# AILab-UniFI/GNN-TableExtraction

Hardware: NVIDIA B200
Metric: page-graphs/sec (fwd+bwd train step) (higher is better)
Workload: dtype f32

## Files before the change

### gnn_tableextraction_b200/csrc/gte_spmm.cu

```cuda
#include "gte_common.cuh"
#include "gte_umma_ptx.cuh"

namespace gte {

template <int VEC>
struct Acc;
template <>
struct Acc<4> {
  float4 v;
  __device__ __forceinline__ void zero() { v = make_float4(0.f, 0.f, 0.f, 0.f); }
  __device__ __forceinline__ void fma(float w, const float4& x) {
    v.x = fmaf(w, x.x, v.x);
    v.y = fmaf(w, x.y, v.y);
    v.z = fmaf(w, x.z, v.z);
    v.w = fmaf(w, x.w, v.w);
  }
};
template <>
struct Acc<1> {
  float v;
  __device__ __forceinline__ void zero() { v = 0.f; }
  __device__ __forceinline__ void fma(float w, float x) { v = fmaf(w, x, v); }
};

// ... 367 lines not shown
    row[q] = (int64_t)cur.n0 + rl;
    if (cur.staged) {
      beg[q] = A.sptr[rl] - cur.e0;
      end[q] = A.sptr[rl + 1] - cur.e0;
    } else {
      beg[q] = __ldg(A.indptr + row[q]) - cur.e0;
      end[q] = __ldg(A.indptr + row[q] + 1) - cur.e0;
    }
  }
  float4 av[R][VV];
  float nrm[R];
#pragma unroll
  for (int q = 0; q < R; ++q) {
#pragma unroll
    for (int v = 0; v < VV; ++v) {
      av[q][v] = make_float4(0.f, 0.f, 0.f, 0.f);
      if (A.addend && on[v]) av[q][v] = __ldg(reinterpret_cast<const float4*>(A.addend + row[q] * A.ldadd + col[v]));
    }
    nrm[q] = 1.0f;
    if (A.mode == GTE_AGG_SUM_NORM) nrm[q] = cur.staged ? A.snrm[rl0 + q * NG] : __ldg(A.row_norm + row[q]);
  }
  float4 acc[R][VV];
#pragma unroll
  for (int q = 0; q < R; ++q)
#pragma unroll
    for (int v = 0; v < VV; ++v) acc[q][v] = make_float4(0.f, 0.f, 0.f, 0.f);
  if (cur.staged) {
    int32_t len = end[0] - beg[0];
    if (R == 2) len = max(len, end[R - 1] - beg[R - 1]);
    auto load_meta = [&](int32_t j, uint2 (&m)[R][U]) {
#pragma unroll
      for (int q = 0; q < R; ++q)
#pragma unroll
        for (int u = 0; u < U; ++u) {
          const int32_t e = beg[q] + j + u;
          m[q][u] = make_uint2(PK_OUTSIDE, 0u);
          if (e < end[q]) m[q][u] = MG ? __ldg(A.gpk + e) : A.spk[e];
        }
    };
    auto step = [&](const uint2 (&m)[R][U]) {
      float4 xv[R][U][VV];
#pragma unroll
      for (int q = 0; q < R; ++q)
#pragma unroll
        for (int u = 0; u < U; ++u) {
          const uint8_t* xr = A.xb + min(m[q][u].x, A.zrow) * ROW_BYTES;
#pragma unroll
          for (int v = 0; v < VV; ++v) xv[q][u][v] = *reinterpret_cast<const float4*>(xr + v * (G * 16));
        }
#pragma unroll
      for (int u = 0; u < U; ++u)
#pragma unroll
        for (int q = 0; q < R; ++q)
#pragma unroll
          for (int v = 0; v < VV; ++v) fma4(acc[q][v], __uint_as_float(m[q][u].y), xv[q][u][v]);
    };
    uint2 ma[R][U], mb[R][U];
    load_meta(0, ma);
    for (int32_t j = 0; j < len; j += 2 * U) {
      load_meta(j + U, mb);
      step(ma);
      if (j + U >= len) break;
      load_meta(j + 2 * U, ma);
      step(mb);
    }
  }
  if (A.slow) {
#pragma unroll 1
    for (int q = 0; q < R; ++q) {
      for (int32_t j = beg[q]; j < end[q]; ++j) {
        const int32_t c = __ldg(A.indices + cur.e0 + j);
        const int32_t sl = c - cur.n0;
        if (cur.staged && sl >= 0 && sl < cur.np) continue;
        float wt = A.w ? __ldg(A.w + (A.eid ? __ldg(A.eid + cur.e0 + j) : cur.e0 + j)) : 1.0f;
        if (A.pre_scale) wt *= __ldg(A.pre_scale + c);
#pragma unroll
        for (int v = 0; v < VV; ++v)
          if (on[v]) {
            const float4 xg = __ldg(reinterpret_cast<const float4*>(A.x + (int64_t)c * A.ldx + col[v]));
            if (q == 0) fma4(acc[0][v], wt, xg);
            else fma4(acc[R - 1][v], wt, xg);
          }
      }
    }
  }
#pragma unroll
  for (int q = 0; q < R; ++q) {
    const int32_t deg = end[q] - beg[q];
    const float d = (float)(deg > 1 ? deg : 1);
#pragma unroll
    for (int v = 0; v < VV; ++v) {
      if (!on[v]) continue;
      float4 r = acc[q][v];
      if (A.mode == GTE_AGG_MEAN) {
        r.x /= d; r.y /= d; r.z /= d; r.w /= d;
      } else if (A.mode == GTE_AGG_SUM_NORM) {
        r.x *= nrm[q]; r.y *= nrm[q]; r.z *= nrm[q]; r.w *= nrm[q];
      }
      if (A.addend) {
        r.x += av[q][v].x; r.y += av[q][v].y; r.z += av[q][v].z; r.w += av[q][v].w;
      }
      *reinterpret_cast<float4*>(A.y + row[q] * A.ldy + col[v]) = r;
    }
  }
}

template <int G, int V, int VV, bool MG>
__device__ __forceinline__ void pk_rows(const PkRowArgs& A) {
  constexpr int NG = PK_CONSUMERS / G;
  const int grp = threadIdx.x / G;
  for (int32_t rl0 = grp; rl0 < A.it.np; rl0 += 2 * NG) {
    if (rl0 + NG < A.it.np)
      pk_row_pass<G, V, VV, 2, MG>(A, rl0);
    else
      pk_row_pass<G, V, VV, 1, MG>(A, rl0);
  }
}

template <int G, int V, bool MG>
__global__ void __launch_bounds__(PK_THREADS, 1)
    k_spmm_paged_pk(const __grid_constant__ PkMaps maps, const int32_t* __restrict__ indptr,
                    const uint2* __restrict__ packed, const int32_t* __restrict__ page_flag,
                    const int32_t* __restrict__ indices, const int32_t* __restrict__ eid, const float* __restrict__ w,
                    const float* __restrict__ pre_scale, const float* __restrict__ row_norm, int mode,
                    const float* __restrict__ x, int64_t ldx, const float* __restrict__ addend, int64_t ldadd,
                    float* __restrict__ y, int64_t ldy, const int32_t* __restrict__ page_off, int32_t f, int32_t num_items,
                    int32_t nslices, int32_t items_per_cta, int32_t np_cap, int32_t ne_cap) {
  extern __shared__ __align__(128) uint8_t pk_smem[];
  constexpr int CS = G * V * 4;
  constexpr int ROW_BYTES = CS * 4;
  const PkStageLayout L = pk_layout(CS, np_cap, MG ? 0 : ne_cap);
  const uint32_t stage_bytes = L.stage_bytes();
  const uint32_t smem0 = (uint32_t)__cvta_generic_to_shared(pk_smem);
  const uint32_t bars = smem0 + 2 * stage_bytes;
  const uint32_t off_pk = L.x_bytes, off_ptr = off_pk + L.pk_bytes, off_nrm = off_ptr + L.ptr_bytes,
                 off_info = off_nrm + L.nrm_bytes;
  const int tid = threadIdx.x;

  const int item_beg = blockIdx.x * items_per_cta;
  const int item_end = min(num_items, item_beg + items_per_cta);
  if (item_beg >= item_end) return;
  if (tid == 0) {
    mbar_init(bars, 2);
    mbar_init(bars + 8, 2);
    mbar_init(bars + 16, PK_CONSUMERS / 32);
    mbar_init(bars + 24, PK_CONSUMERS / 32);
    fence_barrier_init();
    tma_prefetch_desc(&maps.big);
    tma_prefetch_desc(&maps.small);
  }
  for (int i = tid; i < 2 * (ROW_BYTES / 4); i += PK_THREADS) {
    const int st = i / (ROW_BYTES / 4), c = i % (ROW_BYTES / 4);
    reinterpret_cast<float*>(pk_smem + (size_t)st * stage_bytes + L.x_bytes - ROW_BYTES)[c] = 0.f;
  }
  __syncthreads();

  if (tid >= PK_CONSUMERS) {
    const int pl = tid - PK_CONSUMERS;
    auto load_item = [&](int item) {
      PkItem it = {0, 0, 0, 0, 0, 0, 0, 0};
      if (item < item_end) {
        const int page = item / nslices;
        it.c0 = (item - page * nslices) * CS;
        it.n0 = __ldg(page_off + page);
        it.np = __ldg(page_off + page + 1) - it.n0;
        it.e0 = __ldg(indptr + it.n0);
        it.ne = __ldg(indptr + it.n0 + it.np) - it.e0;
        it.flag = __ldg(page_flag + page);
        it.staged = (it.np <= np_cap && (MG || it.ne <= ne_cap)) ? 1 : 0;
      }
      return it;
    };
    PkItem it = load_item(item_beg);
    for (int item = item_beg, s = 0, k = 0; item < item_end; ++item, s ^= 1, ++k) {
      const PkItem nxt = load_item(item + 1);
      if (k >= 2) mbar_wait_backoff(bars + 16 + s * 8, (uint32_t)((k >> 1) - 1) & 1u);
      uint8_t* sbase = pk_smem + (size_t)s * stage_bytes;
      const uint32_t sx = smem0 + s * stage_bytes;
      const uint32_t bar = bars + s * 8;
      if (pl == 0) {
        *reinterpret_cast<PkItem*>(sbase + off_info) = it;
        if (it.staged) {
          const int nbig = it.np / PK_BOX_BIG;
          const int nsmall = (it.np - nbig * PK_BOX_BIG + PK_BOX_SMALL - 1) / PK_BOX_SMALL;
          const int e_lo = it.e0 & ~1;
          const uint32_t pk_copy = (!MG && it.ne > 0) ? (uint32_t)((it.e0 + it.ne - e_lo + 1) & ~1) * 8u : 0u;
          mbar_expect_tx(bar, (uint32_t)(nbig * PK_BOX_BIG + nsmall * PK_BOX_SMALL) * ROW_BYTES + pk_copy);
          for (int b = 0; b < nbig; ++b)
            tma_load_2d(sx + b * PK_BOX_BIG * ROW_BYTES, &maps.big, bar, it.c0, it.n0 + b * PK_BOX_BIG);
          for (int b = 0; b < nsmall; ++b)
            tma_load_2d(sx + (nbig * PK_BOX_BIG + b * PK_BOX_SMALL) * ROW_BYTES, &maps.small, bar, it.c0,
                        it.n0 + nbig * PK_BOX_BIG + b * PK_BOX_SMALL);
          if (pk_copy) bulk_load_1d(sx + off_pk, packed + e_lo, pk_copy, bar);
        } else {
          mbar_arrive(bar);
        }
      }
      if (it.staged) {
        int32_t* sptr = reinterpret_cast<int32_t*>(sbase + off_ptr);
        float* snrm = reinterpret_cast<float*>(sbase + off_nrm);
        const int32_t* ip = indptr + it.n0;
        for (int i = pl; i <= it.np; i += 32) sptr[i] = __ldg(ip + i);
        if (mode == GTE_AGG_SUM_NORM) {
          const float* nr = row_norm + it.n0;
          for (int i = pl; i < it.np; i += 32) snrm[i] = __ldg(nr + i);
        }
      }
      if (addend) {
        for (int i = pl; i < it.np * 2; i += 32) {
          const int col = it.c0 + (i & 1) * 32;
          if (col < f) asm volatile("prefetch.global.L2 [%0];" ::"l"(addend + (int64_t)(it.n0 + (i >> 1)) * ldadd + col));
        }
      }
      __syncwarp();
      if (pl == 0) mbar_arrive(bar);
      it = nxt;
    }
  } else {
    const int lane = tid % G;
    PkRowArgs A;
    A.zrow = L.x_bytes / ROW_BYTES - 1;
    A.indptr = indptr; A.indices = indices; A.eid = eid; A.w = w; A.pre_scale = pre_scale; A.row_norm = row_norm;
    A.mode = mode; A.x = x; A.ldx = ldx; A.addend = addend; A.ldadd = ldadd; A.y = y; A.ldy = ldy; A.f = f;
    for (int item = item_beg, s = 0, k = 0; item < item_end; ++item, s ^= 1, ++k) {
      mbar_wait(bars + s * 8, (uint32_t)(k >> 1) & 1u);
      const uint8_t* sbase = pk_smem + (size_t)s * stage_bytes;
      A.it = *reinterpret_cast<const PkItem*>(sbase + off_info);
      A.xb = sbase + lane * 16;
      A.spk = reinterpret_cast<const uint2*>(sbase + off_pk) + (A.it.e0 & 1);
      A.gpk = packed + A.it.e0;
      A.sptr = reinterpret_cast<const int32_t*>(sbase + off_ptr);
      A.snrm = reinterpret_cast<const float*>(sbase + off_nrm);
      A.slow = !A.it.staged || A.it.flag != 0;
      if (V == 2 && A.it.c0 + G * 4 >= f)
        pk_rows<G, V, 1, MG>(A);
      else
        pk_rows<G, V, V, MG>(A);
      __syncwarp();
      if ((tid & 31) == 0) mbar_arrive(bars + 16 + s * 8);
    }
  }
}

static size_t pk_smem_bytes(int cs, int32_t np_cap, int32_t ne_cap) {
  return 2 * (size_t)pk_layout(cs, np_cap, ne_cap).stage_bytes() + 32;
}

constexpr size_t PK_SMEM_MAX = 227 * 1024;

static void pk_pick(int32_t f, int32_t np_cap, int32_t ne_cap, int* G, int* V, int* MG) {
  const int fv = (f + 3) / 4;
  *G = 0;
  *V = 0;
  *MG = 0;
  struct Cand { int cs, mg; };
  const Cand wide[] = {{64, 0}, {32, 0}, {64, 1}, {32, 1}, {16, 0}, {16, 1}};
  const Cand mid[] = {{32, 0}, {32, 1}, {16, 0}, {16, 1}};
  const Cand narrow[] = {{16, 0}, {16, 1}};
  const Cand* c = fv > 8 ? wide : (fv > 4 ? mid : narrow);
  const int nc = fv > 8 ? 6 : (fv > 4 ? 4 : 2);
  for (int i = 0; i < nc; ++i) {
    if (pk_smem_bytes(c[i].cs, np_cap, c[i].mg ? 0 : ne_cap) <= PK_SMEM_MAX) {
      *G = c[i].cs == 16 ? 4 : 8;
      *V = c[i].cs == 64 ? 2 : 1;
      *MG = c[i].mg;
      return;
    }
  }
}

template <int G, int V, bool MG>
static int launch_spmm_paged_pk(const int32_t* indptr, const uint2* packed, const int32_t* page_flag,
                                const int32_t* indices, const int32_t* eid, const float* w, const float* pre_scale,
                                const float* row_norm, int mode, const float* x, int64_t ldx, const float* addend,
                                int64_t ldadd, float* y, int64_t ldy, const int32_t* page_off, int32_t num_pages,
                                int32_t np_cap, int32_t ne_cap, int32_t n_rows, int32_t f, cudaStream_t st) {
  constexpr int CS = G * V * 4;
  const size_t smem = pk_smem_bytes(CS, np_cap, MG ? 0 : ne_cap);
  if (int rc = ensure_dynamic_smem(reinterpret_cast<const void*>(&k_spmm_paged_pk<G, V, MG>), smem, "k_spmm_paged_pk")) return rc;
  int occ = 1;
  GTE_CHECK_CUDA(cudaOccupancyMaxActiveBlocksPerMultiprocessor(&occ, k_spmm_paged_pk<G, V, MG>, PK_THREADS, smem),
                 "k_spmm_paged_pk(occupancy)");
  if (occ < 1) occ = 1;
  PkMaps maps;
  {
    int rc = make_tmap_2d(&maps.big, x, n_rows, f, ldx, CS, PK_BOX_BIG, CU_TENSOR_MAP_SWIZZLE_NONE);
    if (rc) return rc;
    rc = make_tmap_2d(&maps.small, x, n_rows, f, ldx, CS, PK_BOX_SMALL, CU_TENSOR_MAP_SWIZZLE_NONE);
    if (rc) return rc;
  }
  const int nslices = (int)ceil_div64((f + 3) / 4, G * V);
  const int64_t items = (int64_t)num_pages * nslices;
  GTE_CHECK_ARG(items < (int64_t)1 << 31, "gte_spmm_paged_packed: too many (page, slice) items");
  int grid = (int)(items < (int64_t)sm_count() * occ ? items : (int64_t)sm_count() * occ);
  const int per = (int)ceil_div64(items, grid);
  grid = (int)ceil_div64(items, per);
  k_spmm_paged_pk<G, V, MG><<<grid, PK_THREADS, smem, st>>>(maps, indptr, packed, page_flag, indices, eid, w, pre_scale, row_norm,
                                                       mode, x, ldx, addend, ldadd, y, ldy, page_off, f, (int32_t)items,
                                                       nslices, per, np_cap, ne_cap);
  GTE_CHECK_LAUNCH("k_spmm_paged_pk");
  return GTE_OK;
}

}

using namespace gte;

extern "C" int gte_spmm(const int32_t* indptr, const int32_t* indices, const float* w, const float* pre_scale,
                        const float* row_norm, int mode, const float* x, int64_t ldx, const float* addend,
                        int64_t ldadd, float* y, int64_t ldy, int32_t n_rows, int32_t f, gte_stream_t stream) {
  GTE_CHECK_ARG(n_rows >= 0 && f >= 0, "gte_spmm: negative size");
  GTE_CHECK_ARG(mode == GTE_AGG_SUM || mode == GTE_AGG_SUM_NORM || mode == GTE_AGG_MEAN, "gte_spmm: bad mode %d", mode);
  if (n_rows == 0 || f == 0) return GTE_OK;
  GTE_CHECK_ARG(indptr && indices && x && y, "gte_spmm: null argument");
  GTE_CHECK_ARG(mode != GTE_AGG_SUM_NORM || row_norm, "gte_spmm: SUM_NORM needs row_norm");
  GTE_CHECK_ARG(ldx >= f && ldy >= f && (!addend || ldadd >= f), "gte_spmm: leading dimension < f");
  GTE_CHECK_ARG(x != y, "gte_spmm: x and y must not alias");
  cudaStream_t st = as_stream(stream);
  const bool vec = aligned16(x) && aligned16(y) && (ldx % 4 == 0) && (ldy % 4 == 0) &&
                   (!addend || (aligned16(addend) && ldadd % 4 == 0));
#define GTE_SPMM_GO(VEC, G, C) \
  return launch_spmm<VEC, G, C>(indptr, indices, w, pre_scale, row_norm, mode, x, ldx, addend, ldadd, y, ldy, n_rows, f, st)
  if (vec) {
    const int nv = (f + 3) / 4;
    if (nv <= 4) GTE_SPMM_GO(4, 4, 1);
    if (nv <= 8) GTE_SPMM_GO(4, 8, 1);
    if (nv <= 16) GTE_SPMM_GO(4, 16, 1);
    if (nv <= 32) GTE_SPMM_GO(4, 32, 1);
    if (nv <= 64) GTE_SPMM_GO(4, 32, 2);
    if (nv <= 96) GTE_SPMM_GO(4, 32, 3);
    GTE_SPMM_GO(4, 32, 4);
  } else {
    if (f <= 4) GTE_SPMM_GO(1, 4, 1);
    if (f <= 8) GTE_SPMM_GO(1, 8, 1);
    if (f <= 16) GTE_SPMM_GO(1, 16, 1);
    if (f <= 32) GTE_SPMM_GO(1, 32, 1);
    if (f <= 64) GTE_SPMM_GO(1, 32, 2);
    GTE_SPMM_GO(1, 32, 4);
  }
#undef GTE_SPMM_GO
}

extern "C" int gte_spmm_paged(const int32_t* indptr, const int32_t* indices, const float* w, const float* pre_scale,
                              const float* row_norm, int mode, const float* x, int64_t ldx, const float* addend,
                              int64_t ldadd, float* y, int64_t ldy, const int32_t* page_off, int32_t num_pages,
                              int32_t max_page_nodes, int32_t max_page_edges, int32_t n_rows, int32_t f,
                              gte_stream_t stream) {
  GTE_CHECK_ARG(n_rows >= 0 && f >= 0 && num_pages >= 0 && max_page_nodes >= 0 && max_page_edges >= 0,
                "gte_spmm_paged: negative size");
  GTE_CHECK_ARG(mode == GTE_AGG_SUM || mode == GTE_AGG_SUM_NORM || mode == GTE_AGG_MEAN, "gte_spmm_paged: bad mode %d", mode);
  if (n_rows == 0 || f == 0 || num_pages == 0) return GTE_OK;
  GTE_CHECK_ARG(indptr && indices && x && y && page_off, "gte_spmm_paged: null argument");
  GTE_CHECK_ARG(mode != GTE_AGG_SUM_NORM || row_norm, "gte_spmm_paged: SUM_NORM needs row_norm");
  GTE_CHECK_ARG(ldx >= f && ldy >= f && (!addend || ldadd >= f), "gte_spmm_paged: leading dimension < f");
  GTE_CHECK_ARG(x != y, "gte_spmm_paged: x and y must not alias");
  const bool vec = aligned16(x) && aligned16(y) && (ldx % 4 == 0) && (ldy % 4 == 0) &&
                   (!addend || (aligned16(addend) && ldadd % 4 == 0));
  const size_t budget = 110 * 1024;
  int G = 0;
  const int fv = (f + 3) / 4;
  for (int g : {32, 16, 8}) {
    if (paged_smem_bytes(g, max_page_nodes, max_page_edges) <= budget) {
      G = g;
      break;
    }
  }
  while (G > 8 && G / 2 >= fv) G /= 2;
  if (!vec || G == 0)
    return gte_spmm(indptr, indices, w, pre_scale, row_norm, mode, x, ldx, addend, ldadd, y, ldy, n_rows, f, stream);
  cudaStream_t st = as_stream(stream);
#define GTE_PAGED_GO(GG)                                                                                               \
  return launch_spmm_paged<GG>(indptr, indices, w, pre_scale, row_norm, mode, x, ldx, addend, ldadd, y, ldy, page_off, \
                               num_pages, max_page_nodes, max_page_edges, f, st)
  if (G == 32) GTE_PAGED_GO(32);
  if (G == 16) GTE_PAGED_GO(16);
  GTE_PAGED_GO(8);
#undef GTE_PAGED_GO
}

extern "C" int gte_paged_pack_edges(const int32_t* indptr, const int32_t* indices, const int32_t* eid, const float* w,
                                    const float* pre_scale, const int32_t* page_off, int32_t num_pages,
                                    uint64_t* packed, int32_t* page_flag, gte_stream_t stream) {
  GTE_CHECK_ARG(num_pages >= 0, "gte_paged_pack_edges: negative size");
  if (num_pages == 0) return GTE_OK;
  GTE_CHECK_ARG(indptr && indices && page_off && packed && page_flag, "gte_paged_pack_edges: null argument");
  GTE_CHECK_ARG((reinterpret_cast<uintptr_t>(packed) & 7u) == 0, "gte_paged_pack_edges: packed must be 8-byte aligned");
  k_paged_pack_edges<<<num_pages, 256, 0, as_stream(stream)>>>(indptr, indices, eid, w, pre_scale, page_off,
                                                              reinterpret_cast<uint2*>(packed), page_flag);
  GTE_CHECK_LAUNCH("k_paged_pack_edges");
  return GTE_OK;
}

extern "C" size_t gte_spmm_paged_packed_smem_bytes(int32_t max_page_nodes, int32_t max_page_edges, int32_t f) {
  if (max_page_nodes < 0 || max_page_edges < 0 || f <= 0) return 0;
  int G, V, MG;
  pk_pick(f, max_page_nodes, max_page_edges, &G, &V, &MG);
  return G ? pk_smem_bytes(G * V * 4, max_page_nodes, MG ? 0 : max_page_edges) : 0;
}

extern "C" int gte_spmm_paged_packed(const int32_t* indptr, const uint64_t* packed, const int32_t* page_flag,
                                     const int32_t* indices, const int32_t* eid, const float* w, const float* pre_scale,
                                     const float* row_norm, int mode, const float* x, int64_t ldx, const float* addend,
                                     int64_t ldadd, float* y, int64_t ldy, const int32_t* page_off, int32_t num_pages,
                                     int32_t max_page_nodes, int32_t max_page_edges, int32_t n_rows, int32_t f,
                                     gte_stream_t stream) {
  GTE_CHECK_ARG(n_rows >= 0 && f >= 0 && num_pages >= 0 && max_page_nodes >= 0 && max_page_edges >= 0,
                "gte_spmm_paged_packed: negative size");
  GTE_CHECK_ARG(mode == GTE_AGG_SUM || mode == GTE_AGG_SUM_NORM || mode == GTE_AGG_MEAN, "gte_spmm_paged_packed: bad mode %d",
                mode);
  if (n_rows == 0 || f == 0 || num_pages == 0) return GTE_OK;
  GTE_CHECK_ARG(indptr && packed && page_flag && indices && x && y && page_off, "gte_spmm_paged_packed: null argument");
  GTE_CHECK_ARG(mode != GTE_AGG_SUM_NORM || row_norm, "gte_spmm_paged_packed: SUM_NORM needs row_norm");
  GTE_CHECK_ARG(ldx >= f && ldy >= f && (!addend || ldadd >= f), "gte_spmm_paged_packed: leading dimension < f");
  GTE_CHECK_ARG(x != y, "gte_spmm_paged_packed: x and y must not alias");
  const bool vec = aligned16(x) && aligned16(y) && (ldx % 4 == 0) && (ldy % 4 == 0) &&
                   (!addend || (aligned16(addend) && ldadd % 4 == 0));
  int G, V, MG;
  pk_pick(f, max_page_nodes, max_page_edges, &G, &V, &MG);
  if (!vec || G == 0)
    return fail(GTE_ERR_UNSUPPORTED,
                "gte_spmm_paged_packed: operands not 16-byte aligned or pages too large to stage (query "
                "gte_spmm_paged_packed_smem_bytes first); use gte_spmm_paged");
  cudaStream_t st = as_stream(stream);
  const uint2* pk = reinterpret_cast<const uint2*>(packed);
#define GTE_PK_GO(GG, VV, MM)                                                                                              \
  return launch_spmm_paged_pk<GG, VV, MM>(indptr, pk, page_flag, indices, eid, w, pre_scale, row_norm, mode, x, ldx,     \
                                          addend, ldadd, y, ldy, page_off, num_pages, max_page_nodes, max_page_edges,    \
                                          n_rows, f, st)
  if (G == 8 && V == 2 && !MG) GTE_PK_GO(8, 2, false);
  if (G == 8 && V == 2) GTE_PK_GO(8, 2, true);
  if (G == 8 && !MG) GTE_PK_GO(8, 1, false);
  if (G == 8) GTE_PK_GO(8, 1, true);
  if (!MG) GTE_PK_GO(4, 1, false);
  GTE_PK_GO(4, 1, true);
#undef GTE_PK_GO
}
```

### gnn_tableextraction_b200/csrc/gte_umma2.cu

```cuda
#include "gte_umma_args.cuh"

#include <cuda.h>

namespace gte {

#ifdef GTE_EXPERIMENTS
__device__ long long g_umma2_dbg[148 * 16 * 8];
__device__ long long g_umma2_acc[148 * 16];
#define U2_T0() const long long t0__ = clock64()
#define U2_ACC(var) var += clock64() - t0__
#define U2_PUT(slot, v) do { if (blockIdx.x < 148) g_umma2_acc[blockIdx.x * 16 + (slot)] = (v); } while (0)
#else
#define U2_T0()
#define U2_ACC(var)
#define U2_PUT(slot, v)
#endif

constexpr int U2_THREADS = 448;
constexpr int U2_EPI_WARP0 = 4;
constexpr int U2_EPI_WARPS = 8;
constexpr int U2_SPLIT_WARPS = 4;
constexpr int U2_PREFETCH = 8;
constexpr int U2_EPI_BUF = 4096;
constexpr int U2_MAX_STAGES = 6;
constexpr size_t U2_SMEM_MAX = 227 * 1024;

struct U2Layout {
  uint32_t bh_bytes, stage_bytes, epi_off, par_off, stat_off, bar_off, tmem_off, total;
};
__host__ __device__ inline U2Layout u2_layout(int BN, int stages, int epi_bufs) {
  U2Layout L;
  L.bh_bytes = (uint32_t)(BN / 2) * 128u;
  L.stage_bytes = 2u * UM_A_BYTES + 2u * L.bh_bytes;
  L.epi_off = (uint32_t)stages * L.stage_bytes;
  L.par_off = L.epi_off + U2_EPI_WARPS * U2_EPI_BUF * (uint32_t)epi_bufs;
  L.stat_off = L.par_off + 3u * UM_MAX_BN * 4u;
  L.bar_off = L.stat_off + 2u * 2u * 128u * 8u;
  L.tmem_off = L.bar_off + (3u * U2_MAX_STAGES + 4u) * 8u;
  L.total = L.tmem_off + 16u;
  return L;
}

template <bool SPLIT>
__global__ void __cluster_dims__(2, 1, 1) __launch_bounds__(U2_THREADS, 1)
    k_umma_gemm_pair(const __grid_constant__ UmmaArgs P) {
  extern __shared__ __align__(1024) uint8_t smem_raw[];
  uint8_t* base = smem_raw + ((1024u - (smem_u32(smem_raw) & 1023u)) & 1023u);
  const U2Layout L = u2_layout(P.BN, P.stages, P.epi_bufs);
  const int S = P.stages;
  uint8_t* const tiles = base;
  auto sA_hi_p = [&](int s) { return tiles + s * L.stage_bytes; };
  auto sA_lo_p = [&](int s) { return tiles + s * L.stage_bytes + UM_A_BYTES; };
  auto sB_hi_p = [&](int s) { return tiles + s * L.stage_bytes + 2 * UM_A_BYTES; };
  auto sB_lo_p = [&](int s) { return tiles + s * L.stage_bytes + 2 * UM_A_BYTES + L.bh_bytes; };
  uint8_t* const s_stage = base + L.epi_off;
  float* const s_bias = reinterpret_cast<float*>(base + L.par_off);
  float* const s_gamma = s_bias + UM_MAX_BN;
  float* const s_beta = s_gamma + UM_MAX_BN;
  float2* const s_stat = reinterpret_cast<float2*>(base + L.stat_off);
  uint64_t* const bars = reinterpret_cast<uint64_t*>(base + L.bar_off);
  uint64_t* const bar_full = bars;
  uint64_t* const bar_ready = bars + U2_MAX_STAGES;
  uint64_t* const bar_empty = bars + 2 * U2_MAX_STAGES;
  uint64_t* const bar_tfull = bars + 3 * U2_MAX_STAGES;
  uint64_t* const bar_tempty = bar_tfull + 2;
  uint32_t* const s_tmem = reinterpret_cast<uint32_t*>(base + L.tmem_off);

  const uint32_t rank = cluster_ctarank();
  const int warp = threadIdx.x >> 5;
  const int lane = threadIdx.x & 31;
  const int m_tiles = (P.M + UM_BM - 1) / UM_BM;
  const int m_pairs = (m_tiles + 1) / 2;
  const int total = m_pairs * P.ngroups;
  const int cluster_id = blockIdx.x >> 1, nclusters = gridDim.x >> 1;
  const int kb_total = P.kblocks[0] + (P.nseg > 1 ? P.kblocks[1] : 0);
#ifdef GTE_EXPERIMENTS
  auto stamp = [&](int t, int slot) {
    if (P.dbg && blockIdx.x < 148) {
      const int i = (t - cluster_id) / nclusters;
      if (i < 16) g_umma2_dbg[(blockIdx.x * 16 + i) * 8 + slot] = clock64();
    }
  };
#else
  auto stamp = [](int, int) {};
#endif

  for (int i = threadIdx.x; i < UM_MAX_BN; i += U2_THREADS) {
    s_bias[i] = (P.bias && i < P.bias_n) ? P.bias[i] : 0.f;
    s_gamma[i] = (P.gamma && i < P.N) ? P.gamma[i] : 1.f;
    s_beta[i] = (P.beta && i < P.N) ? P.beta[i] : 0.f;
  }
  if (warp == 0 && lane == 0) {
    for (int s = 0; s < S; ++s) {
      mbar_init(smem_u32(&bar_full[s]), 1);
      mbar_init(smem_u32(&bar_ready[s]), 2 * U2_SPLIT_WARPS);
      mbar_init(smem_u32(&bar_empty[s]), 1);
    }
    for (int a = 0; a < 2; ++a) {
      mbar_init(smem_u32(&bar_tfull[a]), 1);
      mbar_init(smem_u32(&bar_tempty[a]), SPLIT ? 2 * U2_EPI_WARPS : U2_EPI_WARPS);
    }
    fence_barrier_init();
    for (int s = 0; s < P.nseg; ++s) tma_prefetch_desc(&P.tmA[s]);
    for (int gq = 0; gq < P.ngroups; ++gq)
      for (int s = 0; s < P.nseg; ++s) {
        tma_prefetch_desc(&P.tmBhi[gq][s]);
        tma_prefetch_desc(&P.tmBlo[gq][s]);
      }
  }
  if (warp == 1) tmem_alloc_pair(smem_u32(s_tmem), 512);
  tc_fence_before();
  __syncthreads();
  cluster_sync_all();
  tc_fence_after();
  const uint32_t tmem_base = *s_tmem;

  if (warp == 0) {
    if (lane == 0) {
      int stage = 0;
      uint32_t phase = 0;
      const int b_row0 = (int)rank * (P.BN >> 1);
      int pf_t = cluster_id, pf_seg = 0, pf_kb = 0;
      auto pf_step = [&]() {
        if (pf_t >= total) return;
        tma_prefetch_2d(&P.tmA[pf_seg], pf_kb * UM_BK, (2 * (pf_t / P.ngroups) + (int)rank) * UM_BM);
        if (++pf_kb >= P.kblocks[pf_seg]) {
          pf_kb = 0;
          if (++pf_seg >= P.nseg) {
            pf_seg = 0;
            pf_t += nclusters;
          }
        }
      };
#ifdef GTE_EXPERIMENTS
      if (P.dbg & 32) pf_t = total;
#endif
      for (int i = 0; i < U2_PREFETCH; ++i) pf_step();
      long long w_pe = 0, n_kb = 0;
      const long long t_begin = clock64();
      (void)w_pe; (void)n_kb; (void)t_begin;
      for (int t = cluster_id; t < total; t += nclusters) {
        const int mt = 2 * (t / P.ngroups) + (int)rank, grp = t % P.ngroups;
        stamp(t, 7);
        for (int seg = 0; seg < P.nseg; ++seg) {
          for (int kb = 0; kb < P.kblocks[seg]; ++kb) {
            pf_step();
            ++n_kb;
            {
              U2_T0();
              mbar_wait_cluster_backoff(smem_u32(&bar_empty[stage]), phase ^ 1);
              U2_ACC(w_pe);
            }
            const uint32_t fb = smem_u32(&bar_full[stage]);
            mbar_expect_tx(fb, (uint32_t)UM_A_BYTES + 2u * L.bh_bytes);
            tma_load_2d(smem_u32(sA_hi_p(stage)), &P.tmA[seg], fb, kb * UM_BK, mt * UM_BM);
            tma_load_2d(smem_u32(sB_hi_p(stage)), &P.tmBhi[grp][seg], fb, kb * UM_BK, b_row0);
            tma_load_2d(smem_u32(sB_lo_p(stage)), &P.tmBlo[grp][seg], fb, kb * UM_BK, b_row0);
            if (++stage == S) { stage = 0; phase ^= 1; }
          }
        }
      }
      U2_PUT(0, clock64() - t_begin);
      U2_PUT(1, w_pe);
      U2_PUT(9, n_kb);
    }
  } else if (warp == 1) {
    if (rank == 0 && lane == 0) {
      const uint32_t idesc = (1u << 4) | (2u << 7) | (2u << 10) | ((uint32_t)(P.BN >> 3) << 17) | ((uint32_t)(256 >> 4) << 24);
      int stage = 0;
      uint32_t phase = 0;
      int acc = 0;
      uint32_t acc_phase = 0;
      constexpr int nacc = SPLIT ? 1 : 2;
      long long w_mt = 0, w_mr = 0;
      const long long t_begin = clock64();
      (void)w_mt; (void)w_mr; (void)t_begin;
      for (int t = cluster_id; t < total; t += nclusters) {
        stamp(t, 4);
        {
          U2_T0();
          mbar_wait_cluster(smem_u32(&bar_tempty[acc]), acc_phase ^ 1);
          U2_ACC(w_mt);
        }
        tc_fence_after();
        stamp(t, 5);
        const uint32_t d_tmem = tmem_base + (uint32_t)(acc * UM_ACC_STRIDE);
        const uint32_t d_cross = SPLIT ? tmem_base + UM_ACC_STRIDE : d_tmem;
        for (int kb = 0; kb < kb_total; ++kb) {
          {
            U2_T0();
            mbar_wait_cluster(smem_u32(&bar_ready[stage]), phase);
            U2_ACC(w_mr);
          }
          tc_fence_after();
          const uint64_t dah = make_desc_k_sw128(smem_u32(sA_hi_p(stage)));
          const uint64_t dal = make_desc_k_sw128(smem_u32(sA_lo_p(stage)));
          const uint64_t dbh = make_desc_k_sw128(smem_u32(sB_hi_p(stage)));
          const uint64_t dbl = make_desc_k_sw128(smem_u32(sB_lo_p(stage)));
#pragma unroll
          for (int k = 0; k < UM_BK / 8; ++k) {
            const uint64_t adv = (uint64_t)((k * 8 * 4) >> 4);
            umma_tf32_pair(d_cross, dal + adv, dbh + adv, idesc, (kb | k) != 0 ? 1u : 0u);
            umma_tf32_pair(d_cross, dah + adv, dbl + adv, idesc, 1u);
            umma_tf32_pair(d_tmem, dah + adv, dbh + adv, idesc, (SPLIT && (kb | k) == 0) ? 0u : 1u);
          }
          umma_commit_pair(smem_u32(&bar_empty[stage]));
          if (++stage == S) { stage = 0; phase ^= 1; }
        }
        stamp(t, 6);
        umma_commit_pair(smem_u32(&bar_tfull[acc]));
        if (++acc == nacc) { acc = 0; acc_phase ^= 1; }
      }
      U2_PUT(4, w_mt);
      U2_PUT(5, w_mr);
      U2_PUT(6, clock64() - t_begin);
    }
  } else if (warp < U2_EPI_WARP0 || warp >= U2_EPI_WARP0 + U2_EPI_WARPS) {
    const int t = ((warp < U2_EPI_WARP0) ? warp - 2 : warp - (U2_EPI_WARP0 + U2_EPI_WARPS) + 2) * 32 + lane;
    const uint32_t ready_leader = mapa_shared(smem_u32(&bar_ready[0]), 0);
    int stage = 0;
    uint32_t phase = 0;
    long long w_sf = 0, w_sw = 0;
    (void)w_sf; (void)w_sw;
    for (int tile = cluster_id; tile < total; tile += nclusters) {
      for (int kb = 0; kb < kb_total; ++kb) {
        {
          U2_T0();
          mbar_wait_backoff(smem_u32(&bar_full[stage]), phase);
          U2_ACC(w_sf);
        }
        U2_T0();
        const float4* hi = reinterpret_cast<const float4*>(sA_hi_p(stage));
        float4* lo = reinterpret_cast<float4*>(sA_lo_p(stage));
#pragma unroll
        for (int i = 0; i < UM_A_BYTES / 16 / (U2_SPLIT_WARPS * 32); ++i) {
          const int idx = t + U2_SPLIT_WARPS * 32 * i;
          const float4 v = hi[idx];
          float4 l;
          l.x = tf32_rna(v.x - tf32_hi(v.x)); l.y = tf32_rna(v.y - tf32_hi(v.y));
          l.z = tf32_rna(v.z - tf32_hi(v.z)); l.w = tf32_rna(v.w - tf32_hi(v.w));
          lo[idx] = l;
        }
        fence_proxy_async();
        __syncwarp();
        if (lane == 0) mbar_arrive_cluster(ready_leader + (uint32_t)stage * 8u);
        U2_ACC(w_sw);
        if (++stage == S) { stage = 0; phase ^= 1; }
      }
    }
    if (t == 0) {
      U2_PUT(2, w_sf);
      U2_PUT(3, w_sw);
    }
  } else {
    const int ew = warp - U2_EPI_WARP0;
    const int q = warp & 3;
    const int half = ew >> 2;
    uint8_t* const stb = s_stage + ew * U2_EPI_BUF * P.epi_bufs;
    const int nbuf = P.epi_bufs;
    const uint32_t tempty_leader = mapa_shared(smem_u32(&bar_tempty[0]), 0);
    int store_seq = 0;
    int acc = 0;
    uint32_t acc_phase = 0;
    int par = 0;
    constexpr int nacc = SPLIT ? 1 : 2;
    const int nchunks = (P.N + 31) / 32;
    const int c_split = SPLIT ? (nchunks + 1) / 2 : nchunks;
    const int c_beg = (SPLIT && half) ? c_split : 0, c_end = (SPLIT && half) ? nchunks : c_split;
    const int cols_a = min(P.N, c_split * 32);
    const float n_a = (float)cols_a, n_b = (float)(P.N - cols_a), n_all = (float)P.N;
    const float my_n = (SPLIT && half) ? n_b : n_a;
    long long w_et = 0, w_ew = 0;
    (void)w_et; (void)w_ew;
    int it = 0;
    for (int t = cluster_id; t < total; t += nclusters, ++it) {
      const int mt = 2 * (t / P.ngroups) + (int)rank, grp = t % P.ngroups;
      if constexpr (!SPLIT) {
        if ((it & 1) != half) continue;
        acc = half;
        acc_phase = (uint32_t)(it >> 1) & 1u;
      }
      if (ew == 0 && lane == 0) stamp(t, 0);
      {
        U2_T0();
        mbar_wait_cluster_backoff(smem_u32(&bar_tfull[acc]), acc_phase);
        U2_ACC(w_et);
      }
      U2_T0();
      tc_fence_after();
      if (ew == 0 && lane == 0) stamp(t, 1);
      const uint32_t t_base = tmem_base + ((uint32_t)(q * 32) << 16) + (uint32_t)(acc * UM_ACC_STRIDE);
      const int64_t row0 = (int64_t)mt * UM_BM + q * 32;
      const bool rows_live = row0 < (int64_t)P.M;
      const bool store_z = P.out[grp] != nullptr && rows_live;
      const bool store_y = P.y != nullptr && rows_live;
      float x[32];
      const int rows_valid = rows_live ? (int)min((int64_t)32, (int64_t)P.M - row0) : 0;
      auto put_chunk = [&](const CUtensorMap* map, float* dst, int64_t ld, int c) {
#ifdef GTE_EXPERIMENTS
        if (P.dbg & 2) return;
#endif
        if (P.tma_store == 2)
          epi_store_chunk_lsu(stb, x, dst + row0 * ld + c * 32, ld, rows_valid, P.N - c * 32);
        else
          epi_store_chunk_tma(stb, nbuf, store_seq, x, map, c * 32, (int32_t)row0);
      };
#define load_chunk(c) epi_load_chunk<SPLIT>(t_base + (c) * 32, s_bias + (c) * 32, x)
      if (P.fuse_ln) {
        float shift = 0.f, s1 = 0.f, s2 = 0.f;
        for (int c = c_beg; c < c_end; ++c) {
          load_chunk(c);
          const int nv = min(32, P.N - c * 32);
          if (c == c_beg) {
            float s0 = 0.f;
#pragma unroll
            for (int j = 0; j < 32; ++j) s0 += (j < nv) ? x[j] : 0.f;
            shift = s0 / (float)nv;
          }
#ifdef GTE_EXPERIMENTS
          if (P.dbg & 8) { s1 += x[0]; s2 += x[1]; } else
#endif
          if (nv == 32) {
#pragma unroll
            for (int j = 0; j < 32; ++j) {
              const float d = x[j] - shift;
              s1 += d;
              s2 = fmaf(d, d, s2);
            }
          } else {
#pragma unroll
            for (int j = 0; j < 32; ++j) {
              const float d = (j < nv) ? x[j] - shift : 0.f;
              s1 += d;
              s2 = fmaf(d, d, s2);
            }
          }
          if (store_z) put_chunk(&P.tmOut[grp], P.out[grp], P.ldo[grp], c);
        }
        float mh = 0.f, m2h = 0.f;
        if (my_n > 0.f) {
          mh = shift + s1 / my_n;
          m2h = fmaxf(s2 - s1 * s1 / my_n, 0.f);
        }
        float mean = mh, m2 = m2h;
        if constexpr (SPLIT) {
          float2* const st = s_stat + (par * 2) * 128 + q * 32 + lane;
          st[half * 128] = make_float2(mh, m2h);
          asm volatile("bar.sync %0, 64;" ::"r"(1 + q) : "memory");
          const float2 pa = st[0], pb = st[128];
          par ^= 1;
          mean = pa.x;
          m2 = pa.y;
          if (n_b > 0.f) {
            const float delta = pb.x - pa.x;
            mean = pa.x + delta * (n_b / n_all);
            m2 = pa.y + pb.y + delta * delta * (n_a * n_b / n_all);
          }
        }
        const float rstd = 1.0f / sqrtf(m2 / n_all + P.eps);
        if (!SPLIT || half == 0) {
          const int64_t grow = row0 + lane;
          if (grow < P.M) {
            P.mean[grow] = mean;
            P.rstd[grow] = rstd;
          }
        }
        if (ew == 0 && lane == 0) stamp(t, 2);
        for (int c = c_beg; c < c_end; ++c) {
          load_chunk(c);
#ifdef GTE_EXPERIMENTS
          if (!(P.dbg & 4))
#endif
          epi_norm_act(x, s_gamma + c * 32, s_beta + c * 32, true, P.relu != 0, mean, rstd);
          if (store_y) put_chunk(&P.tmY, P.y, P.ldy, c);
        }
      } else {
        if (ew == 0 && lane == 0) stamp(t, 2);
        for (int c = c_beg; c < c_end; ++c) {
          load_chunk(c);
          if (store_z) put_chunk(&P.tmOut[grp], P.out[grp], P.ldo[grp], c);
          if (P.y != nullptr) {
            epi_norm_act(x, s_gamma + c * 32, s_beta + c * 32, false, P.relu != 0, 0.f, 1.f);
            if (store_y) put_chunk(&P.tmY, P.y, P.ldy, c);
          }
        }
      }
#undef load_chunk
      if (ew == 0 && lane == 0) stamp(t, 3);
      tc_fence_before();
      __syncwarp();
      if (lane == 0) mbar_arrive_cluster(tempty_leader + (uint32_t)acc * 8u);
      if constexpr (SPLIT) {
        if (++acc == nacc) { acc = 0; acc_phase ^= 1; }
      }
      U2_ACC(w_ew);
    }
    if (ew == 0 && lane == 0) {
      U2_PUT(7, w_et);
      U2_PUT(8, w_ew);
    }
    if (lane == 0) tma_store_wait_all();
  }
  tc_fence_before();
  __syncwarp();
  __syncthreads();
  cluster_sync_all();
  if (warp == 1) {
    tc_fence_after();
    tmem_dealloc_pair(tmem_base, 512);
  }
}

static void u2_pick(int BN, int kb_total, int* stages, int* epi_bufs) {
  *stages = 0;
  *epi_bufs = 1;
  if (kb_total <= 2) {
    for (int b = 4; b >= 1; --b)
      if (1024 + (size_t)u2_layout(BN, 2, b).total <= U2_SMEM_MAX) {
        *stages = 2;
        *epi_bufs = b;
        return;
      }
    return;
  }
  for (int s = U2_MAX_STAGES; s >= 2; --s)
    if (1024 + (size_t)u2_layout(BN, s, 1).total <= U2_SMEM_MAX) {
      *stages = s;
      if (1024 + (size_t)u2_layout(BN, s, 2).total <= U2_SMEM_MAX) *epi_bufs = 2;
      return;
    }
}

bool umma_pair_supported(const UmmaArgs& a) {
  const int m_tiles = (a.M + UM_BM - 1) / UM_BM;
  int st = 0, eb = 0;
  u2_pick(a.BN, 3, &st, &eb);
  return a.tma_store != 0 && m_tiles >= 2 && a.BN % 16 == 0 && a.BN >= 16 && a.BN <= UM_MAX_BN && sm_count() >= 2 && st >= 2;
}

int launch_umma_pair(UmmaArgs& a, cudaStream_t st) {
  if (int rc = setup_weight_maps(a, a.BN / 2)) return rc;
  const int kb_total = a.kblocks[0] + (a.nseg > 1 ? a.kblocks[1] : 0);
  int stages = 0, epi_bufs = 1;
  u2_pick(a.BN, kb_total, &stages, &epi_bufs);
  if (stages < 2) return fail(GTE_ERR_UNSUPPORTED, "k_umma_gemm_pair: BN=%d does not fit shared memory", a.BN);
  a.stages = stages;
  a.epi_bufs = epi_bufs;
  if (tuning(GTE_TUNE_EPI_STORE) == 1) a.tma_store = 2;
  const size_t smem = 1024 + (size_t)u2_layout(a.BN, a.stages, a.epi_bufs).total;
  if (int rc = ensure_dynamic_smem(reinterpret_cast<const void*>(&k_umma_gemm_pair<true>), smem, "k_umma_gemm_pair")) return rc;
  if (int rc = ensure_dynamic_smem(reinterpret_cast<const void*>(&k_umma_gemm_pair<false>), smem, "k_umma_gemm_pair")) return rc;
  const int m_tiles = (a.M + UM_BM - 1) / UM_BM;
  const int total = ((m_tiles + 1) / 2) * a.ngroups;
  int clusters = sm_count() / 2;
  if (clusters > total) clusters = total;
  if (clusters < 1) return GTE_OK;
  if (kb_total > 2 && tuning(GTE_TUNE_UMMA_SPLIT) != 0)
    k_umma_gemm_pair<true><<<2 * clusters, U2_THREADS, smem, st>>>(a);
  else
    k_umma_gemm_pair<false><<<2 * clusters, U2_THREADS, smem, st>>>(a);
  GTE_CHECK_LAUNCH("k_umma_gemm_pair");
  return GTE_OK;
}

int umma_pair_debug_times(int64_t* out_host, int32_t count) {
#ifdef GTE_EXPERIMENTS
  if (count == 148 * 16) {
    GTE_CHECK_CUDA(cudaMemcpyFromSymbol(out_host, g_umma2_acc, (size_t)count * 8), "gte_umma_debug_times");
    return GTE_OK;
  }
  GTE_CHECK_CUDA(cudaMemcpyFromSymbol(out_host, g_umma2_dbg, (size_t)count * 8), "gte_umma_debug_times");
  return GTE_OK;
#else
  (void)out_host;
  (void)count;
  return fail(GTE_ERR_UNSUPPORTED, "built without -DGTE_EXPERIMENTS");
#endif
}

}
```

Before: 390,900.

## Add narrow-feature paged SpMM kernel and grouped 128-row TMA epilogue stores

Adds a dedicated SpMM kernel for feature widths up to 16 that stages a whole page's node features, packed edges and row pointers into shared memory with cp.async. Each node row is then handled by four threads using float4 lanes, which avoids the wider slice-based packed kernel that wastes lanes on narrow features. Separately, the paired UMMA GEMM epilogue gains a grouped TMA store mode: the four epilogue warps write a swizzled 128x32 tile and one thread issues the store after a named barrier. This replaces per-warp 32-row stores and rebuilds the output tensor maps with a 128-row box. The costs are an extra barrier in the epilogue and a different shared-buffer indexing scheme.

```diff
diff --git a/gnn_tableextraction_b200/csrc/gte_spmm.cu b/gnn_tableextraction_b200/csrc/gte_spmm.cu
--- a/gnn_tableextraction_b200/csrc/gte_spmm.cu
+++ b/gnn_tableextraction_b200/csrc/gte_spmm.cu
@@ -693,6 +693,155 @@
   return GTE_OK;
 }
 
+constexpr int NW_THREADS = 256;
+constexpr int NW_ROWS = NW_THREADS / 4;
+
+struct NwLayout {
+  uint32_t x_bytes, pk_bytes, ptr_bytes;
+  __host__ __device__ uint32_t total() const { return x_bytes + pk_bytes + ptr_bytes; }
+};
+__host__ __device__ inline NwLayout nw_layout(int32_t np_cap, int32_t ne_cap) {
+  NwLayout l;
+  l.x_bytes = ((uint32_t)np_cap + 1) * 64;
+  l.pk_bytes = (uint32_t)ne_cap * 8;
+  l.ptr_bytes = (((uint32_t)np_cap + 1) * 4 + 15u) & ~15u;
+  return l;
+}
+
+__device__ __forceinline__ void cp_async_16_zfill(void* dst, const void* src, uint32_t src_bytes) {
+  asm volatile("cp.async.cg.shared.global [%0], [%1], 16, %2;" ::"r"((uint32_t)__cvta_generic_to_shared(dst)), "l"(src),
+               "r"(src_bytes)
+               : "memory");
+}
+__device__ __forceinline__ void cp_async_8(void* dst, const void* src) {
+  asm volatile("cp.async.ca.shared.global [%0], [%1], 8;" ::"r"((uint32_t)__cvta_generic_to_shared(dst)), "l"(src) : "memory");
+}
+__device__ __forceinline__ void cp_async_4(void* dst, const void* src) {
+  asm volatile("cp.async.ca.shared.global [%0], [%1], 4;" ::"r"((uint32_t)__cvta_generic_to_shared(dst)), "l"(src) : "memory");
+}
+
+__global__ void __launch_bounds__(NW_THREADS)
+    k_spmm_narrow(const int32_t* __restrict__ indptr, const uint2* __restrict__ packed, const int32_t* __restrict__ page_flag,
+                  const int32_t* __restrict__ indices, const int32_t* __restrict__ eid, const float* __restrict__ w,
+                  const float* __restrict__ pre_scale, const float* __restrict__ row_norm, int mode,
+                  const float* __restrict__ x, int64_t ldx, const float* __restrict__ addend, int64_t ldadd,
+                  float* __restrict__ y, int64_t ldy, const int32_t* __restrict__ page_off, int32_t f, int32_t np_cap,
+                  int32_t ne_cap) {
+  extern __shared__ __align__(16) uint8_t nw_smem[];
+  const NwLayout L = nw_layout(np_cap, ne_cap);
+  float4* sx = reinterpret_cast<float4*>(nw_smem);
+  uint2* spk = reinterpret_cast<uint2*>(nw_smem + L.x_bytes);
+  int32_t* sptr = reinterpret_cast<int32_t*>(nw_smem + L.x_bytes + L.pk_bytes);
+  const int tid = threadIdx.x;
+  const int page = blockIdx.x;
+  const int32_t n0 = __ldg(page_off + page), np = __ldg(page_off + page + 1) - n0;
+  const int32_t e0 = __ldg(indptr + n0), ne = __ldg(indptr + n0 + np) - e0;
+  const bool staged = np <= np_cap && ne <= ne_cap;
+  const bool slow = !staged || __ldg(page_flag + page) != 0;
+  if (staged) {
+    for (int i = tid; i < np * 4; i += NW_THREADS) {
+      const int r = i >> 2, c = (i & 3) * 4;
+      const int valid = min(max(f - c, 0), 4);
+      cp_async_16_zfill(sx + i, x + (int64_t)(n0 + r) * ldx + (valid ? c : 0), (uint32_t)valid * 4u);
+    }
+    for (int i = tid; i < ne; i += NW_THREADS) cp_async_8(spk + i, packed + e0 + i);
+    for (int i = tid; i <= np; i += NW_THREADS) cp_async_4(sptr + i, indptr + n0 + i);
+    asm volatile("cp.async.commit_group;" ::: "memory");
+    if (tid < 4) sx[np_cap * 4 + tid] = make_float4(0.f, 0.f, 0.f, 0.f);
+  }
+  const int lane = tid & 3;
+  const int col = lane * 4;
+  const bool on = col < f;
+  const uint32_t zrow = (uint32_t)np_cap;
+  auto row_ops = [&](int32_t rl, float4& a, float& nr) {
+    a = make_float4(0.f, 0.f, 0.f, 0.f);
+    nr = 1.0f;
+    if (rl >= np) return;
+    const int64_t row = (int64_t)n0 + rl;
+    if (addend && on) a = __ldg(reinterpret_cast<const float4*>(addend + row * ldadd + col));
+    if (mode == GTE_AGG_SUM_NORM) nr = __ldg(row_norm + row);
+  };
+  float4 av_next;
+  float nrm_next;
+  row_ops(tid >> 2, av_next, nrm_next);
+  if (staged) asm volatile("cp.async.wait_group 0;" ::: "memory");
+  __syncthreads();
+
+  for (int32_t rl = tid >> 2; rl < np; rl += NW_ROWS) {
+    const int64_t row = (int64_t)n0 + rl;
+    const float4 av = av_next;
+    const float nrm = nrm_next;
+    row_ops(rl + NW_ROWS, av_next, nrm_next);
+    int32_t beg, end;
+    if (staged) {
+      beg = sptr[rl] - e0;
+      end = sptr[rl + 1] - e0;
+    } else {
+      beg = __ldg(indptr + row) - e0;
+      end = __ldg(indptr + row + 1) - e0;
+    }
+    float4 acc = make_float4(0.f, 0.f, 0.f, 0.f);
+    if (staged) {
+      int32_t j = beg;
+      for (; j + 4 <= end; j += 4) {
+        const uint2 m0 = spk[j], m1 = spk[j + 1], m2 = spk[j + 2], m3 = spk[j + 3];
+        const float4 x0 = sx[min(m0.x, zrow) * 4 + lane];
+        const float4 x1 = sx[min(m1.x, zrow) * 4 + lane];
+        const float4 x2 = sx[min(m2.x, zrow) * 4 + lane];
+        const float4 x3 = sx[min(m3.x, zrow) * 4 + lane];
+        fma4(acc, __uint_as_float(m0.y), x0);
+        fma4(acc, __uint_as_float(m1.y), x1);
+        fma4(acc, __uint_as_float(m2.y), x2);
+        fma4(acc, __uint_as_float(m3.y), x3);
+      }
+      for (; j < end; ++j) {
+        const uint2 m = spk[j];
+        fma4(acc, __uint_as_float(m.y), sx[min(m.x, zrow) * 4 + lane]);
+      }
+    }
+    if (slow && on) {
+      for (int32_t j = beg; j < end; ++j) {
+        const int32_t c = __ldg(indices + e0 + j);
+        const int32_t sl = c - n0;
+        if (staged && sl >= 0 && sl < np) continue;
+        float wt = w ? __ldg(w + (eid ? __ldg(eid + e0 + j) : e0 + j)) : 1.0f;
+        if (pre_scale) wt *= __ldg(pre_scale + c);
+        fma4(acc, wt, __ldg(reinterpret_cast<const float4*>(x + (int64_t)c * ldx + col)));
+      }
+    }
+    if (!on) continue;
+    if (mode == GTE_AGG_MEAN) {
+      const int32_t deg = end - beg;
+      const float d = (float)(deg > 1 ? deg : 1);
+      acc.x /= d; acc.y /= d; acc.z /= d; acc.w /= d;
+    } else if (mode == GTE_AGG_SUM_NORM) {
+      acc.x *= nrm; acc.y *= nrm; acc.z *= nrm; acc.w *= nrm;
+    }
+    if (addend) {
+      acc.x += av.x; acc.y += av.y; acc.z += av.z; acc.w += av.w;
+    }
+    *reinterpret_cast<float4*>(y + row * ldy + col) = acc;
+  }
+}
+
+static size_t nw_smem_bytes(int32_t np_cap, int32_t ne_cap) {
+  if ((int64_t)np_cap * 64 + (int64_t)ne_cap * 8 > (int64_t)PK_SMEM_MAX) return 0;
+  const size_t b = nw_layout(np_cap, ne_cap).total();
+  return b <= PK_SMEM_MAX ? b : 0;
+}
+
+static int launch_spmm_narrow(const int32_t* indptr, const uint2* packed, const int32_t* page_flag, const int32_t* indices,
+                              const int32_t* eid, const float* w, const float* pre_scale, const float* row_norm, int mode,
+                              const float* x, int64_t ldx, const float* addend, int64_t ldadd, float* y, int64_t ldy,
+                              const int32_t* page_off, int32_t num_pages, int32_t np_cap, int32_t ne_cap, int32_t f,
+                              size_t smem, cudaStream_t st) {
+  if (int rc = ensure_dynamic_smem(reinterpret_cast<const void*>(&k_spmm_narrow), smem, "k_spmm_narrow")) return rc;
+  k_spmm_narrow<<<num_pages, NW_THREADS, smem, st>>>(indptr, packed, page_flag, indices, eid, w, pre_scale, row_norm, mode,
+                                                     x, ldx, addend, ldadd, y, ldy, page_off, f, np_cap, ne_cap);
+  GTE_CHECK_LAUNCH("k_spmm_narrow");
+  return GTE_OK;
+}
+
 }
 
 using namespace gte;
@@ -784,6 +933,9 @@
 
 extern "C" size_t gte_spmm_paged_packed_smem_bytes(int32_t max_page_nodes, int32_t max_page_edges, int32_t f) {
   if (max_page_nodes < 0 || max_page_edges < 0 || f <= 0) return 0;
+  if (f <= 16) {
+    if (const size_t b = nw_smem_bytes(max_page_nodes, max_page_edges)) return b;
+  }
   int G, V, MG;
   pk_pick(f, max_page_nodes, max_page_edges, &G, &V, &MG);
   return G ? pk_smem_bytes(G * V * 4, max_page_nodes, MG ? 0 : max_page_edges) : 0;
@@ -806,14 +958,19 @@
   GTE_CHECK_ARG(x != y, "gte_spmm_paged_packed: x and y must not alias");
   const bool vec = aligned16(x) && aligned16(y) && (ldx % 4 == 0) && (ldy % 4 == 0) &&
                    (!addend || (aligned16(addend) && ldadd % 4 == 0));
+  cudaStream_t st = as_stream(stream);
+  const uint2* pk = reinterpret_cast<const uint2*>(packed);
+  if (f <= 16 && vec) {
+    if (const size_t smem = nw_smem_bytes(max_page_nodes, max_page_edges))
+      return launch_spmm_narrow(indptr, pk, page_flag, indices, eid, w, pre_scale, row_norm, mode, x, ldx, addend, ldadd,
+                                y, ldy, page_off, num_pages, max_page_nodes, max_page_edges, f, smem, st);
+  }
   int G, V, MG;
   pk_pick(f, max_page_nodes, max_page_edges, &G, &V, &MG);
   if (!vec || G == 0)
     return fail(GTE_ERR_UNSUPPORTED,
                 "gte_spmm_paged_packed: operands not 16-byte aligned or pages too large to stage (query "
                 "gte_spmm_paged_packed_smem_bytes first); use gte_spmm_paged");
-  cudaStream_t st = as_stream(stream);
-  const uint2* pk = reinterpret_cast<const uint2*>(packed);
 #define GTE_PK_GO(GG, VV, MM)                                                                                              \
   return launch_spmm_paged_pk<GG, VV, MM>(indptr, pk, page_flag, indices, eid, w, pre_scale, row_norm, mode, x, ldx,     \
                                           addend, ldadd, y, ldy, page_off, num_pages, max_page_nodes, max_page_edges,    \
diff --git a/gnn_tableextraction_b200/csrc/gte_umma2.cu b/gnn_tableextraction_b200/csrc/gte_umma2.cu
--- a/gnn_tableextraction_b200/csrc/gte_umma2.cu
+++ b/gnn_tableextraction_b200/csrc/gte_umma2.cu
@@ -39,6 +39,29 @@
   L.tmem_off = L.bar_off + (3u * U2_MAX_STAGES + 4u) * 8u;
   L.total = L.tmem_off + 16u;
   return L;
+}
+
+__device__ __forceinline__ void epi_store_group_tma(uint8_t* gbufs, int nbuf, int& seq, const float (&v)[32],
+                                                    const CUtensorMap* map, int32_t col0, int32_t row0, int q, int bar_id) {
+  const int lane = threadIdx.x & 31;
+  uint8_t* buf = gbufs + (seq % nbuf) * (4 * U2_EPI_BUF);
+  float* rowp = reinterpret_cast<float*>(buf + q * U2_EPI_BUF) + lane * 32;
+#pragma unroll
+  for (int k = 0; k < 8; ++k)
+    *reinterpret_cast<float4*>(rowp + ((k ^ (lane & 7)) << 2)) = make_float4(v[4 * k], v[4 * k + 1], v[4 * k + 2], v[4 * k + 3]);
+  fence_proxy_async();
+  const bool issuer = q == 0 && lane == 0;
+  if (issuer) {
+    if (nbuf == 2) tma_store_wait_read<0>();
+    else if (nbuf == 3) tma_store_wait_read<1>();
+    else tma_store_wait_read<2>();
+  }
+  asm volatile("bar.sync %0, 128;" ::"r"(bar_id) : "memory");
+  if (issuer) {
+    tma_store_2d(map, smem_u32(buf), col0, row0);
+    tma_store_commit();
+  }
+  ++seq;
 }
 
 template <bool SPLIT>
@@ -257,6 +280,7 @@
     const int q = warp & 3;
     const int half = ew >> 2;
     uint8_t* const stb = s_stage + ew * U2_EPI_BUF * P.epi_bufs;
+    uint8_t* const gstb = s_stage + half * 4 * U2_EPI_BUF * P.epi_bufs;
     const int nbuf = P.epi_bufs;
     const uint32_t tempty_leader = mapa_shared(smem_u32(&bar_tempty[0]), 0);
     int store_seq = 0;
@@ -292,8 +316,10 @@
       const uint32_t t_base = tmem_base + ((uint32_t)(q * 32) << 16) + (uint32_t)(acc * UM_ACC_STRIDE);
       const int64_t row0 = (int64_t)mt * UM_BM + q * 32;
       const bool rows_live = row0 < (int64_t)P.M;
-      const bool store_z = P.out[grp] != nullptr && rows_live;
-      const bool store_y = P.y != nullptr && rows_live;
+      const bool group_store = !SPLIT && P.tma_store == 3;
+      const bool live = group_store ? (int64_t)mt * UM_BM < (int64_t)P.M : rows_live;
+      const bool store_z = P.out[grp] != nullptr && live;
+      const bool store_y = P.y != nullptr && live;
       float x[32];
       const int rows_valid = rows_live ? (int)min((int64_t)32, (int64_t)P.M - row0) : 0;
       auto put_chunk = [&](const CUtensorMap* map, float* dst, int64_t ld, int c) {
@@ -302,6 +328,8 @@
 #endif
         if (P.tma_store == 2)
           epi_store_chunk_lsu(stb, x, dst + row0 * ld + c * 32, ld, rows_valid, P.N - c * 32);
+        else if (group_store)
+          epi_store_group_tma(gstb, nbuf, store_seq, x, map, c * 32, mt * UM_BM, q, 5 + half);
         else
           epi_store_chunk_tma(stb, nbuf, store_seq, x, map, c * 32, (int32_t)row0);
       };
@@ -447,6 +475,15 @@
   a.stages = stages;
   a.epi_bufs = epi_bufs;
   if (tuning(GTE_TUNE_EPI_STORE) == 1) a.tma_store = 2;
+  const bool split = kb_total > 2 && tuning(GTE_TUNE_UMMA_SPLIT) != 0;
+  if (!split && a.tma_store == 1 && epi_bufs >= 2) {
+    for (int g = 0; g < a.ngroups; ++g)
+      if (a.out[g] != nullptr)
+        if (int rc = make_tmap_2d(&a.tmOut[g], a.out[g], a.M, a.N, a.ldo[g], 32, UM_BM)) return rc;
+    if (a.y != nullptr)
+      if (int rc = make_tmap_2d(&a.tmY, a.y, a.M, a.N, a.ldy, 32, UM_BM)) return rc;
+    a.tma_store = 3;
+  }
   const size_t smem = 1024 + (size_t)u2_layout(a.BN, a.stages, a.epi_bufs).total;
   if (int rc = ensure_dynamic_smem(reinterpret_cast<const void*>(&k_umma_gemm_pair<true>), smem, "k_umma_gemm_pair")) return rc;
   if (int rc = ensure_dynamic_smem(reinterpret_cast<const void*>(&k_umma_gemm_pair<false>), smem, "k_umma_gemm_pair")) return rc;
@@ -455,7 +492,7 @@
   int clusters = sm_count() / 2;
   if (clusters > total) clusters = total;
   if (clusters < 1) return GTE_OK;
-  if (kb_total > 2 && tuning(GTE_TUNE_UMMA_SPLIT) != 0)
+  if (split)
     k_umma_gemm_pair<true><<<2 * clusters, U2_THREADS, smem, st>>>(a);
   else
     k_umma_gemm_pair<false><<<2 * clusters, U2_THREADS, smem, st>>>(a);
```

New measurement: 397,700, median of 6. 1.02x the previous value.
